# vearch/gamma

Hardware: AMD Instinct MI355X
Metric: queries/sec @ recall@10>=0.95, IVFPQ nlist=4096 nprobe=32 (higher is better)
Workload: dtype f32

## Files before the change

gamma_amd/_lib.py:

```python
import ctypes as C
import os

HERE = os.path.dirname(os.path.abspath(__file__))
LIB_PATH = os.path.join(HERE, "libgamma_hip.so")

f32p = C.POINTER(C.c_float)
i64p = C.POINTER(C.c_int64)
i32p = C.POINTER(C.c_int32)
u8p = C.POINTER(C.c_uint8)

NUM_STAGES = 6
STAGE_NAMES = ["coarse", "tables", "scan", "select", "rerank", "flat"]


class RangeFilter(C.Structure):
    _fields_ = [("bitmap", u8p), ("bitmap_bytes", C.c_int64), ("min_doc", C.c_int32),
                ("max_doc", C.c_int32), ("min_aligned", C.c_int32), ("b_not_in", C.c_int32)]


class FieldFilter(C.Structure):
    _fields_ = [("field_id", C.c_int32), ("include_lower", C.c_int32), ("include_upper", C.c_int32),
                ("reserved", C.c_int32), ("lower_i", C.c_int64), ("upper_i", C.c_int64),
                ("lower_f", C.c_double), ("upper_f", C.c_double)]

# ... 36 lines not shown
    "gamma_hip_raw_i8_check": (C.c_int, [f32p, C.c_int64, C.c_int, i64p]),
    "gamma_hip_raw_init_sq8": (C.c_int, [C.c_void_p, C.c_int]),
    "gamma_hip_raw_sq8_set_ranges": (C.c_int, [C.c_void_p, f32p, f32p]),
    "gamma_hip_raw_sq8_get_ranges": (C.c_int, [C.c_void_p, f32p, f32p]),
    "gamma_hip_raw_sq8_train": (C.c_int, [C.c_void_p, C.c_int64, f32p]),
    "gamma_hip_raw_sq8_check": (C.c_int, [f32p, C.c_int64, i64p]),
    "gamma_hip_raw_sq8_params": (C.c_int, [C.c_int, f32p, f32p, f32p, f32p]),
    "gamma_hip_raw_append": (C.c_int, [C.c_void_p, C.c_int64, f32p]),
    "gamma_hip_raw_update": (C.c_int, [C.c_void_p, C.c_int64, f32p]),
    "gamma_hip_ivfpq_arena_stats": (C.c_int, [C.c_void_p, i64p]),
    "gamma_hip_ivfpq_arena_growth": (C.c_int, [C.c_void_p, i64p]),
    "gamma_hip_ivfpq_set_repack_threshold": (C.c_int, [C.c_void_p, C.c_int64]),
    "gamma_hip_set_small_path": (C.c_int, [C.c_void_p, C.c_int]),
    "gamma_hip_set_flat_narrow_rows": (C.c_int, [C.c_void_p, C.c_int]),
    "gamma_hip_set_ivfflat_narrow_rows": (C.c_int, [C.c_void_p, C.c_int]),
    "gamma_hip_ivfflat_lm_shape": (C.c_int, [C.c_int, C.POINTER(C.c_int), C.POINTER(C.c_int), C.POINTER(C.c_int)]),
    "gamma_hip_ivfflat_scan_stats": (C.c_int, [C.c_void_p, i64p, C.c_int]),
    "gamma_hip_set_flat_sq8_rows": (C.c_int, [C.c_void_p, C.c_int]),
    "gamma_hip_set_ivfflat_sq8_rows": (C.c_int, [C.c_void_p, C.c_int]),
    "gamma_hip_set_coarse_fused": (C.c_int, [C.c_void_p, C.c_int, C.c_int]),
    "gamma_hip_coarse_filter_stats": (C.c_int, [C.c_void_p, i64p]),
    "gamma_hip_set_rerank_filter": (C.c_int, [C.c_void_p, C.c_int]),
    "gamma_hip_rerank_filter_stats": (C.c_int, [C.c_void_p, i64p]),
    "gamma_hip_flat_filter_shape": (C.c_int, [C.c_int, C.POINTER(C.c_int), C.POINTER(C.c_float)]),
    "gamma_hip_flat_filter_stats": (C.c_int, [C.c_void_p, i64p, C.c_int]),
    "gamma_hip_tie_stats": (C.c_int, [C.c_void_p, i64p, C.c_int]),
    "gamma_hip_ties_not_honoured": (C.c_int, [C.c_void_p, i64p, C.c_int]),
    "gamma_hip_blas_form_not_restated": (C.c_int, [C.c_void_p, i64p, C.c_int]),
    "gamma_hip_raw_write": (C.c_int, [C.c_void_p, C.c_int64, C.c_int64, f32p]),
    "gamma_hip_raw_gets": (C.c_int, [C.c_void_p, C.c_int64, i64p, f32p]),
    "gamma_hip_ivfpq_repack_verify_stats": (C.c_int, [C.c_void_p, i64p]),
    "gamma_hip_raw_count": (C.c_int64, [C.c_void_p]),
    "gamma_hip_raw_stats": (C.c_int, [C.c_void_p, i64p]),
    "gamma_hip_bitmap_upload": (C.c_int, [C.c_void_p, u8p, C.c_int64]),
    "gamma_hip_bitmap_set": (C.c_int, [C.c_void_p, i64p, C.c_int64, C.c_int]),
    "gamma_hip_ivfpq_init": (C.c_int, [C.c_void_p] + [C.c_int] * 7),
    "gamma_hip_ivfpq4_init": (C.c_int, [C.c_void_p] + [C.c_int] * 6),
    "gamma_hip_opq_set": (C.c_int, [C.c_void_p, f32p]),
    "gamma_hip_opq_get": (C.c_int, [C.c_void_p, f32p]),
    "gamma_hip_opq_apply": (C.c_int, [C.c_void_p, C.c_int64, f32p, f32p]),
    "gamma_hip_opq_apply_device": (C.c_int, [C.c_void_p, C.c_int64, C.c_void_p, C.c_void_p]),
    "gamma_hip_opq_train": (C.c_int, [C.c_void_p, C.c_int, C.c_int64, f32p, C.c_int, C.c_int, f32p, C.POINTER(C.c_float)]),
    "gamma_hip_ivfpq_set_trained": (C.c_int, [C.c_void_p, f32p, f32p, f32p]),
    "gamma_hip_ivfpq_get_precomputed_table": (C.c_int, [C.c_void_p, f32p]),
    "gamma_hip_set_precomputed_table_max_bytes": (C.c_int, [C.c_int64]),
    "gamma_hip_get_precomputed_table_max_bytes": (C.c_int64, []),
# ... 185 lines not shown
```

gamma_amd/api.py:

```python
import ctypes as C

import numpy as np

from . import _lib
from ._lib import GammaHipError, RangeFilter, SearchParams

METRIC_IP = 0
METRIC_L2 = 1

FLT_TINY = float(np.finfo(np.float32).tiny)
FLT_MAX = float(np.finfo(np.float32).max)


def _f32(a):
    return np.ascontiguousarray(a, dtype=np.float32)


def _p(a, t):
    return a.ctypes.data_as(t) if a is not None else None


def make_range_filter(docids, b_not_in=False):
    docids = np.asarray(sorted(set(int(x) for x in docids)), dtype=np.int64)
    mn, mx = (int(docids[0]), int(docids[-1])) if len(docids) else (0, 0)
# ... 641 lines not shown
        out = np.zeros(4, np.int64)
        self._ck(self.L.gamma_hip_scan_bound_stats(self.h, _p(out, _lib.i64p)), "scan_bound_stats")
        return dict(zip(["fell_through", "queries", "backoffs", "gave_up_waiting"], [int(v) for v in out]))

    def set_dist_budget(self, nbytes):
        self._ck(self.L.gamma_hip_set_workspace_budget(self.h, int(nbytes)), "set_workspace_budget")

    def set_coarse_fused(self, on=True, list_cap=128):
        self._ck(self.L.gamma_hip_set_coarse_fused(self.h, int(on), list_cap), "set_coarse_fused")

    def coarse_filter_stats(self):
        out = np.zeros(4, np.int64)
        self._ck(self.L.gamma_hip_coarse_filter_stats(self.h, _p(out, _lib.i64p)), "coarse_filter_stats")
        return dict(zip(["given_up", "queries", "backoffs", "fp32_calls_left"], [int(v) for v in out]))

    def set_rerank_filter(self, mode=1):
        self._ck(self.L.gamma_hip_set_rerank_filter(self.h, int(mode)), "set_rerank_filter")

    def rerank_filter_stats(self):
        out = np.zeros(5, np.int64)
        self._ck(self.L.gamma_hip_rerank_filter_stats(self.h, _p(out, _lib.i64p)), "rerank_filter_stats")
        return dict(zip(["candidates", "survivors", "calls", "backoffs", "image_rows"], [int(v) for v in out]))

    def flat_filter_stats(self, reset=False):
        out = np.zeros(3, np.int64)
        self._ck(self.L.gamma_hip_flat_filter_stats(self.h, _p(out, _lib.i64p), 1 if reset else 0), "flat_filter_stats")
        return tuple(int(v) for v in out)

    def set_small_path(self, on=True):
        self._ck(self.L.gamma_hip_set_small_path(self.h, int(on)), "set_small_path")

    def set_flat_narrow_rows(self, on=True):
        self._ck(self.L.gamma_hip_set_flat_narrow_rows(self.h, 1 if on else 0), "set_flat_narrow_rows")

    def set_ivfflat_narrow_rows(self, on=True):
        self._ck(self.L.gamma_hip_set_ivfflat_narrow_rows(self.h, 1 if on else 0), "set_ivfflat_narrow_rows")

    def ivfflat_scan_stats(self, reset=False):
        out = np.zeros(4, np.int64)
        self._ck(self.L.gamma_hip_ivfflat_scan_stats(self.h, _p(out, _lib.i64p), 1 if reset else 0), "ivfflat_scan_stats")
        return tuple(int(v) for v in out)

    def set_flat_sq8_rows(self, on=True):
        self._ck(self.L.gamma_hip_set_flat_sq8_rows(self.h, 1 if on else 0), "set_flat_sq8_rows")

    def set_ivfflat_sq8_rows(self, on=True):
# ... 256 lines not shown
```

gamma_amd/csrc/gamma_hip.cpp:

```cpp
#include "gamma_hip_internal.h"

using namespace ghi;

extern "C" {

const char* gamma_hip_strerror(int code) {
    switch (code) {
        case GAMMA_HIP_OK: return "ok";
        case GAMMA_HIP_EINVAL: return "invalid argument";
        case GAMMA_HIP_ENOTTRAINED: return "index not trained";
        case GAMMA_HIP_EDEVICE: return "HIP runtime error";
        case GAMMA_HIP_ENOMEM: return "out of memory";
        case GAMMA_HIP_EFULL: return "inverted list full";
        case GAMMA_HIP_EUNSUPPORTED: return "exact ties requested beyond the replay's range";
        default: return "unknown error";
    }
}

int gamma_hip_create(int device, gamma_hip_index** out) {
    if (!out) return GAMMA_HIP_EINVAL;
    *out = nullptr;
    int ndev = 0;
    if (hipGetDeviceCount(&ndev) != hipSuccess || ndev <= 0) return GAMMA_HIP_EDEVICE;
    if (device < 0 || device >= ndev) return GAMMA_HIP_EINVAL;
// ... 177 lines not shown
    h->rf.mode = mode;
    h->rf.off_calls = 0;
    return GAMMA_HIP_OK;
}

int gamma_hip_rerank_filter_stats(gamma_hip_index* h, int64_t* out5) {
    if (!h || !out5) return GAMMA_HIP_EINVAL;
    SearchLock lk(h);
    std::vector<unsigned long long> v(gh::kRerankFilterStatLines * 16, 0);
    if (h->rf.d_stat) {
        GH_CHECK(h, hipSetDevice(h->device));
        GH_CHECK(h, hipStreamSynchronize(h->stream));
        GH_CHECK(h, hipMemcpy(v.data(), h->rf.d_stat, gh::rerank_filter_stat_bytes(), hipMemcpyDeviceToHost));
    }
    out5[0] = (int64_t)h->rf.cand;
    out5[1] = 0;
    for (int i = 0; i < gh::kRerankFilterStatLines; i++) out5[1] += (int64_t)v[16 * i];
    out5[2] = h->rf.calls;
    out5[3] = h->rf.backoffs;
    out5[4] = h->rf.on ? h->nraw : 0;
    return GAMMA_HIP_OK;
}

int gamma_hip_flat_filter_shape(int d, int* d_pad, float* margin) { return gh::flat_filter_shape(d, d_pad, margin); }

int gamma_hip_flat_filter_stats(gamma_hip_index* h, int64_t* out3, int reset) {
    if (!h || !out3) return GAMMA_HIP_EINVAL;
    out3[0] = reset ? h->ff_passes.exchange(0) : h->ff_passes.load();
    out3[1] = reset ? h->ff_pairs.exchange(0) : h->ff_pairs.load();
    out3[2] = reset ? h->ff_redone.exchange(0) : h->ff_redone.load();
    return GAMMA_HIP_OK;
}

int gamma_hip_ivfflat_lm_shape(int d, int* kind, int* slab, int* qtile) {
    if (!kind || !slab || !qtile) return GAMMA_HIP_EINVAL;
    gh::ivfflat_lm_shape(d, kind, slab, qtile);
    return GAMMA_HIP_OK;
}

int gamma_hip_ivfflat_scan_stats(gamma_hip_index* h, int64_t* out4, int reset) {
    if (!h || !out4) return GAMMA_HIP_EINVAL;
    out4[0] = reset ? h->fl_small.exchange(0) : h->fl_small.load();
    out4[1] = reset ? h->fl_pair.exchange(0) : h->fl_pair.load();
    out4[2] = reset ? h->fl_lm.exchange(0) : h->fl_lm.load();
    out4[3] = reset ? h->fl_lms.exchange(0) : h->fl_lms.load();
    return GAMMA_HIP_OK;
// ... 161 lines not shown
```

gamma_amd/csrc/gamma_hip_internal.h:

```cpp
#pragma once
#include "../../include/gamma_hip.h"

#include <hip/hip_runtime.h>
#include <math.h>
#include <stdlib.h>
#include <string.h>

#include <algorithm>
#include <atomic>
#include <map>
#include <chrono>
#include <condition_variable>
#include <cstring>
#include <deque>
#include <functional>
#include <mutex>
#include <string>
#include <thread>
#include <unordered_map>
#include <vector>

#include "call_slots.h"
#include "dev_mem.h"
#include "kernels.h"
// ... 121 lines not shown
    int64_t raw_cap() const { return raw_d > 0 ? (int64_t)(raw.cap / ((size_t)raw_d * raw_esz())) : 0; }
    std::vector<float> sq8_vmin, sq8_vmax, sq8_step;
    float* d_sq8_tab = nullptr;
    size_t raw_esz() const { return gh::row_elem_bytes(raw_et); }
    bool has_raw_rows() const { return raw.p != nullptr; }
    int raw_elem_type() const { return raw_et; }
    bool raw_narrow() const { return raw_et != gh::ROW_F32; }
    const float* raw_f32() const { return raw_et == gh::ROW_F32 ? static_cast<const float*>(raw.p) : nullptr; }
    float* raw_f32() { return raw_et == gh::ROW_F32 ? static_cast<float*>(raw.p) : nullptr; }
    bool raw_sparse = false;
    std::vector<int32_t> h_raw_slot;
    ghi::DevArrayOf<int32_t> d_raw_slot;
    int64_t raw_slot_cap() const { return (int64_t)(d_raw_slot.cap / sizeof(int32_t)); }
    int64_t raw_live = 0;
    std::vector<int32_t> raw_free;

    struct RerankImage {
        ghi::DevArray rows, aux;
        float* par = nullptr;
        bool on = false;
        hipEvent_t built = nullptr;
        int mode = 1;
        static constexpr int kAutoMinNq = 1024;
        unsigned long long* d_stat = nullptr;
        unsigned long long* pin_stat = nullptr;
        unsigned long long seen[2] = {0, 0};
        unsigned long long cand = 0, cand_at_copy = 0;
        hipEvent_t copy_ev = nullptr;
        bool copy_pending = false;
        uint64_t sig = 0;
        int off_calls = 0;
        int64_t backoffs = 0, calls = 0;
        int64_t cap_rows(int d) const { return d > 0 ? (int64_t)std::min(rows.cap / (size_t)d, aux.cap / (2 * sizeof(float))) : 0; }
    } rf;

    struct Column {
        int dtype = 0;
        ghi::DevArrayOf<uint8_t> d;
        int64_t n = 0;
    };
    std::map<int, Column> fields;
    struct TermColumn {
        ghi::DevArrayOf<int64_t> d_off;
        ghi::DevArrayOf<int32_t> d_tok;
        int64_t ndocs = 0, ntok = 0;
        std::vector<int64_t> h_rows;
// ... 316 lines not shown
```

gamma_amd/csrc/gamma_hip_search.cpp:

```cpp
#include "gamma_hip_internal.h"
#include "gamma_hip_search.h"
#include "opq.h"

namespace ghi {


int build_filter(H* h, const gamma_hip_search_params* p, gh::FilterDesc* f, size_t* off_io, int64_t est_codes) {
    memset(f, 0, sizeof(*f));
    f->del_bitmap = h->d_bitmap;
    f->del_bits = h->d_bitmap ? h->bitmap_bits : 0;
    f->vid2doc = h->h_v2d.empty() ? nullptr : h->d_v2d;
    f->n_vid2doc = (int64_t)h->h_v2d.size();
    f->has_range = p->has_range ? 1 : 0;
    f->n_range = p->has_range ? p->n_range : 0;
    if (f->n_range > gh::kMaxRange) return fail(h, GAMMA_HIP_EINVAL, "too many range filters");
    if (f->n_range > 0) {
        size_t tot = 0;
        for (int i = 0; i < f->n_range; i++) tot += ((size_t)p->range[i].bitmap_bytes + 15) & ~(size_t)15;
        if (!off_io) GH_CHECK(h, h->w_filter.ensure(tot));
        size_t off = off_io ? *off_io : 0;
        for (int i = 0; i < f->n_range; i++) {
            const gamma_hip_range_filter& r = p->range[i];
            uint8_t* dst = h->w_filter.as<uint8_t>() + off;
            GH_CHECK(h, hipMemcpyAsync(dst, r.bitmap, (size_t)r.bitmap_bytes, hipMemcpyHostToDevice,
// ... 725 lines not shown
        a.cand_dis = const_cast<float*>(cand_dis);
        a.cand_ids = const_cast<int64_t*>(cand_ids);
        a.distances = d_distances;
        a.labels = d_labels;
        static const bool no_side = getenv("GAMMA_HIP_NO_SIDE_STREAM") != nullptr;
        if (h->defer_now && h->side2 && !no_side) {
            (void)hipEventRecord(h->ev_rfork, s);
            (void)hipStreamWaitEvent(h->side2, h->ev_rfork, 0);
            gh::launch_tie_replay(h->side2, l2, a);
            (void)hipEventRecord(h->ev_rdone, h->side2);
            h->replay_pending = true;
            h->replay_is_flat = false;
        } else {
            gh::launch_tie_replay(s, l2, a);
        }
    };
    if (p->has_rank) {
        if (!h->has_raw_rows() || h->raw_d != h->d) return fail(h, GAMMA_HIP_EINVAL, "has_rank needs the raw store");
        if (h->raw_sparse) return fail(h, GAMMA_HIP_EUNSUPPORTED, "has_rank on a handle that holds its shard's raw rows only: the exact distances travel with the candidates (gamma_hip_ivfpq_shard_exact / _merge_rerank_exact)");
        if (R <= 1024 && (nq >= 256 || ties)) {
            bool filt = false;
            GH_TRY(rerank_filter_begin(h, l2, nq, R, k, &filt));
            if (filt) {
                gh::launch_rerank_topk_filtered(s, l2, d_x, nq, h->d, h->raw_f32(), h->nraw, h->rf.rows.as<uint8_t>(),
                                                h->rf.aux.as<float>(), h->rf.par, cand_ids, R, k, p->min_score, p->max_score, neutral,
                                                d_distances, d_labels, qperm, ties ? &tf : nullptr, h->rf.d_stat);
                GH_TRY(rerank_filter_end(h, (int64_t)nq * R));
            } else {
                gh::launch_rerank_topk(s, l2, d_x, nq, h->d, raw_rows_ref(h), h->nraw, cand_ids, R, k, p->min_score,
                                       p->max_score, neutral, d_distances, d_labels, qperm, ties ? &tf : nullptr);
            }
            if (ties && tie_mode == 1) replay();
            GH_CHECK(h, hipGetLastError());
            return GAMMA_HIP_OK;
        }
        GH_CHECK(h, h->w_exact.ensure((size_t)nq * R * sizeof(float)));
        GH_CHECK(h, h->w_selv.ensure((size_t)nq * k * sizeof(float)));
        GH_CHECK(h, h->w_selp.ensure((size_t)nq * k * sizeof(int)));
        gh::launch_rerank_dist(s, l2, d_x, nq, h->d, raw_rows_ref(h), h->nraw, cand_ids, R, p->min_score,
                               p->max_score, h->w_exact.as<float>());
        gh::launch_select_topk(s, l2, h->w_exact.as<float>(), R, nullptr, R, R, nq, k,
                               h->w_selv.as<float>(), h->w_selp.as<int>());
        gh::launch_finalize_topk(s, h->w_selv.as<float>(), h->w_selp.as<int>(), nq, k, cand_ids, R, 0,
                                 neutral, d_distances, d_labels);
        if (ties) {
            GH_CHECK(h, h->w_textra.ensure((size_t)nq));
            GH_CHECK(h, hipMemsetAsync(h->w_textra.p, 0, (size_t)nq, s));
            gh::launch_flag_cut_ties(s, h->w_exact.as<float>(), R, nullptr, nq, k, h->w_selv.as<float>(), h->w_selp.as<int>(),
                                     h->w_textra.as<uint8_t>(), R, 1);
// ... 527 lines not shown
```

gamma_amd/csrc/kernels.h:

```cpp
#pragma once
#include <atomic>
#include <hip/hip_runtime.h>
#include <stdint.h>

#include "scan_plan.h"

namespace gh {

void launch_refused(const char* what);
const char* launch_refused_take();


inline bool first_call_on_device(std::atomic<uint64_t>& done) {
    int dev = 0;
    (void)hipGetDevice(&dev);
    const uint64_t bit = 1ull << (dev & 63);
    return (done.fetch_or(bit) & bit) == 0;
}

constexpr int kMaxRange = 8;

struct RangeDesc {
    const uint8_t* bitmap;
    int32_t min_doc, max_doc, min_aligned, b_not_in;
// ... 327 lines not shown
                         const float* vals, const int64_t* ids, int64_t stride, const int32_t* off, int P, const float* bound, float* ex);
void launch_lookup_exact(hipStream_t s, bool l2, const float* all_dis, const int64_t* all_ids, const float* all_exact, int W, int nq, int R,
                         int q0, int nql, const float* cand_dis, const int64_t* cand_ids, float* cand_exact);
struct TieFlags {
    const uint8_t* cut = nullptr;
    int* list = nullptr;
    int* count = nullptr;
    unsigned long long* stats = nullptr;
};
void launch_rerank_topk(hipStream_t s, bool l2, const float* x, int nq, int d, const RowsRef& raw,
                        int64_t nraw, const int64_t* cand_ids, int R, int k, float min_score,
                        float max_score, float neutral, float* distances, int64_t* labels,
                        const int* qperm = nullptr,
                        const TieFlags* ties = nullptr);
constexpr float kRerankFilterMargin = 3.0517578125e-05f;
constexpr int kRerankFilterMaxD = 1536;
constexpr int kRerankFilterStatLines = 64;
inline size_t rerank_filter_stat_bytes() { return (size_t)kRerankFilterStatLines * 16 * sizeof(unsigned long long); }
bool rerank_filter_shape_ok(int d, int R, int k);
inline size_t rerank_image_par_bytes(int d) { return ((size_t)3 * d + 2) * sizeof(float); }
void launch_rerank_image_params(hipStream_t s, const float* rows, int64_t n, int d, float* par);
void launch_rerank_image_rows(hipStream_t s, const float* rows, const int64_t* vids, int64_t first, int64_t n, int d, const float* par,
                              uint8_t* img, float* aux, int64_t nrows);
void launch_rerank_topk_filtered(hipStream_t s, bool l2, const float* x, int nq, int d, const float* raw, int64_t nraw, const uint8_t* img,
                                 const float* aux, const float* par, const int64_t* cand_ids, int R, int k, float min_score,
                                 float max_score, float neutral, float* distances, int64_t* labels, const int* qperm,
                                 const TieFlags* ties, unsigned long long* stat);
struct TieReplayArgs {
    const int* list;
    const int* count;
    int nq;
    const float* slab;
    int64_t q_stride;
    const int* pair_off;
    const int64_t* pair_base;
    const int64_t* ids;
    int P, G;
    const unsigned long long* ready;
    const unsigned long long* surv;
    const int* gcnt;
    int nsl, slice_cap;
    const float* x;
    int d;
    RowsRef rows;
    int64_t nraw;
    const float* ex_slab = nullptr;
    int* ex_missing = nullptr;
    int R, k, has_rank;
    float min_score, max_score, neutral;
    float* cand_dis;
// ... 73 lines not shown
```

gamma_amd/csrc/rerank_filter.hip:

```cpp
#include <hip/hip_runtime.h>
#include <stdint.h>

#include <algorithm>

#include "block_utils.h"
#include "device_math.h"
#include "kernels.h"
#include "rerank_dev.h"
#include "rerank_topk_dev.h"

namespace gh {

namespace {
constexpr float kM = kRerankFilterMargin;

__device__ __forceinline__ float group8_sum(float a) {
    a += __shfl_down(a, 4, 8);
    a += __shfl_down(a, 2, 8);
    return a + __shfl_down(a, 1, 8);
}
__device__ __forceinline__ float byte_f(uint32_t w, int b) { return (float)((w >> (8 * b)) & 0xffu); }

__device__ __forceinline__ float block_sum256(float v, float* red) {
#pragma unroll
    for (int o = 32; o > 0; o >>= 1) v += __shfl_down(v, o, 64);
    __syncthreads();
    if ((threadIdx.x & 63) == 0) red[threadIdx.x >> 6] = v;
    __syncthreads();
    return (red[0] + red[1]) + (red[2] + red[3]);
}
}

__global__ __launch_bounds__(256) void k_img_minmax_init(uint32_t* __restrict__ keys, int d) {
    const int j = blockIdx.x * 256 + threadIdx.x;
    if (j < d) {
        keys[j] = 0xffffffffu;
        keys[d + j] = 0u;
    }
}
__global__ __launch_bounds__(256) void k_img_minmax(const float* __restrict__ rows, int64_t n, int d, uint32_t* __restrict__ keys) {
    __shared__ uint32_t s_lo[4][64], s_hi[4][64];
    const int tx = threadIdx.x & 63, ty = threadIdx.x >> 6;
    const int j = blockIdx.x * 64 + tx;
    uint32_t lo = 0xffffffffu, hi = 0u;
    if (j < d)
        for (int64_t r = (int64_t)blockIdx.y * 4 + ty; r < n; r += (int64_t)gridDim.y * 4) {
            const float v = rows[r * d + j];
            if (fabsf(v) < INFINITY) {
                const uint32_t kk = f2key(v);
                lo = min(lo, kk);
                hi = max(hi, kk);
            }
        }
// ... 100 lines not shown
        launch_refused("launch_rerank_image_rows: d is not a multiple of 16");
        return;
    }
    hipLaunchKernelGGL(k_img_quantise, dim3((unsigned)((n + 31) / 32)), dim3(256), 0, s, rows, vids, first, n, d, par, img,
                       reinterpret_cast<float2*>(aux), nrows);
}

template <bool L2, bool D128>
__global__ __launch_bounds__(256) void k_rerank_topk_filt(const float* __restrict__ x, int d, const float* __restrict__ raw, int64_t nraw,
                                                          const uint8_t* __restrict__ img, const float2* __restrict__ aux,
                                                          const float* __restrict__ par, const int64_t* __restrict__ cand_ids, int R,
                                                          int k, float min_score, float max_score, float neutral,
                                                          float* __restrict__ distances, int64_t* __restrict__ labels, int nq,
                                                          const int* __restrict__ qperm, TieFlags tf,
                                                          unsigned long long* __restrict__ stat) {
    __shared__ unsigned long long s_it[1024];
    __shared__ int64_t s_id[1024];
    __shared__ float s_bd[1024];
    __shared__ unsigned short s_sv[1024];
    __shared__ __attribute__((aligned(16))) float s_x[D128 ? 128 : kRerankFilterMaxD];
    __shared__ float s_red[4];
    __shared__ float s_tau;
    __shared__ int s_tie, s_nsv;
    int q = blockIdx.x;
    if (qperm) {
        const int qi = (blockIdx.x & 7) * ((nq + 7) >> 3) + (blockIdx.x >> 3);
        if (qi >= nq) return;
        q = qperm[qi];
    } else if (q >= nq) {
        return;
    }
    const int l = threadIdx.x & 7, g = threadIdx.x >> 3;
    const float* xq = x + (int64_t)q * d;
    const float sentinel = L2 ? INFINITY : -INFINITY;
    const float delta = par[d], lon = par[d + 1];
    for (int r = threadIdx.x; r < R; r += 256) s_id[r] = cand_ids[(int64_t)q * R + r];
    if (threadIdx.x == 0) s_nsv = 0;
    float sq = 0.f, sc = 0.f;
    for (int j = threadIdx.x; j < d; j += 256) {
        const float xv = xq[j];
        const float v = L2 ? __fsub_rn(xv, par[j]) : xv;
        s_x[j] = v;
        sq = __builtin_fmaf(v, v, sq);
        if (!L2) sc = __builtin_fmaf(xv, par[j], sc);
    }
    const float xn = sqrtf(block_sum256(sq, s_red)) * (1.0f + kM);
    float c0 = 0.f;
    if (!L2) c0 = block_sum256(sc, s_red);

    if constexpr (D128) {
        float xx[16];
#pragma unroll
        for (int u = 0; u < 16; u++) xx[u] = s_x[16 * l + u];
        for (int r0 = 0; r0 < R; r0 += 128) {
            uint4 w[4];
#pragma unroll
            for (int f = 0; f < 4; f++) {
                const int r = r0 + 32 * f + g;
                const int64_t id = r < R ? s_id[r] : -1;
                w[f] = make_uint4(0, 0, 0, 0);
#if GH_RERANK_TIMING == 5
                w[f] = make_uint4((uint32_t)id, l, f, 7);
#else
                if (id >= 0 && id < nraw) w[f] = *reinterpret_cast<const uint4*>(img + id * 128 + 16 * l);
#endif
            }
#pragma unroll
            for (int f = 0; f < 4; f++) {
                const uint32_t ww[4] = {w[f].x, w[f].y, w[f].z, w[f].w};
                float a = 0.f;
#pragma unroll
// ... 24 lines not shown
                    const uint32_t ww[4] = {w.x, w.y, w.z, w.w};
#pragma unroll
                    for (int v = 0; v < 4; v++) {
                        const float4 xv = *reinterpret_cast<const float4*>(s_x + 16 * c + 4 * v);
                        const float xs[4] = {xv.x, xv.y, xv.z, xv.w};
#pragma unroll
                        for (int b = 0; b < 4; b++) {
                            const float uf = byte_f(ww[v], b);
                            if (L2) {
                                const float t = __builtin_fmaf(-delta, uf, xs[b]);
                                a = __builtin_fmaf(t, t, a);
                            } else {
                                a = __builtin_fmaf(xs[b], uf, a);
                            }
                        }
                    }
                }
            }
            a = group8_sum(a);
            if (l == 0 && r < R) s_bd[r] = a;
        }
    }
    __syncthreads();
    float bd[4];
    bool alive[4];
#pragma unroll
    for (int u = 0; u < 4; u++) {
        const int r = threadIdx.x + 256 * u;
        bd[u] = 0.f;
        alive[u] = false;
        if (r < R) {
            const int64_t id = s_id[r];
            const bool live = id >= 0 && id < nraw;
            float2 ax = make_float2(0.f, 0.f);
#if GH_RERANK_TIMING == 2
            if (live) ax = make_float2(0.1f, 1000.0f);
#else
            if (live) ax = aux[id];
#endif
            const float a = s_bd[r];
            float lb, ub;
            if (L2) {
                const float rt = sqrtf(a);
                const float slack = __builtin_fmaf(kM, rt + xn, ax.x);
                const float ur = rt + slack, lr = fmaxf(rt - slack, 0.0f);
                ub = ur * ur * (1.0f + kM);
                lb = lr * lr * (1.0f - kM);
            } else {
                const float est = __builtin_fmaf(delta, a, c0);
                const float slack = xn * __builtin_fmaf(kM, ax.y + lon, ax.x);
                ub = est + slack;
                lb = est - slack;
            }
            const bool inside = live && ub <= max_score && lb >= min_score;
            alive[u] = live && !(lb > max_score || ub < min_score);
            const uint32_t key = L2 ? f2key(ub) : ~f2key(lb);
            s_it[r] = inside ? (((unsigned long long)key << 32) | (unsigned)r) : ~0ull;
            bd[u] = L2 ? lb : ub;
        }
    }
    if (threadIdx.x == 0) {
        if (tf.list) s_tie = tf.cut ? tf.cut[q] : 0;
        s_tau = sentinel;
    }
    const int K1 = min(k + 1, R);
    const bool head = K1 <= 16 && R > 64;
    if (head) {
        __syncthreads();
        if (threadIdx.x < 64) {
            const unsigned long long it = wave_sort64(s_it[threadIdx.x]);
            const uint32_t key = (uint32_t)(it >> 32);
            if ((int)threadIdx.x == K1 - 1 && key != 0xffffffffu) s_tau = key2f(L2 ? key : ~key);
        }
    } else {
        rerank_first_k(s_it, R, K1);
        if (threadIdx.x == 0) {
            const uint32_t key = (uint32_t)(s_it[K1 - 1] >> 32);
            if (key != 0xffffffffu) s_tau = key2f(L2 ? key : ~key);
        }
    }
    __syncthreads();
    const float tau = s_tau;
    const uint32_t skey = L2 ? f2key(sentinel) : ~f2key(sentinel);
    bool sv[4];
#pragma unroll
    for (int u = 0; u < 4; u++) sv[u] = alive[u] && !(L2 ? bd[u] > tau : bd[u] < tau);
#pragma unroll
    for (int u = 0; u < 4; u++) {
        const int r = threadIdx.x + 256 * u;
        if (256 * u < R) {
            const unsigned long long bal = __ballot(sv[u]);
            const int lane = threadIdx.x & 63;
            int base = 0;
            if (lane == 0 && bal) base = atomicAdd(&s_nsv, __popcll(bal));
            base = __shfl(base, 0, 64);
            if (sv[u]) s_sv[base + __popcll(bal & ((1ull << lane) - 1ull))] = (unsigned short)r;
            else if (r < R) s_it[r] = ((unsigned long long)skey << 32) | (unsigned)r;
        }
    }
    __syncthreads();
#if GH_RERANK_TIMING == 3
    const int m = 0;
#else
    const int m = s_nsv;
#endif
#if GH_RERANK_TIMING != 4
    if (threadIdx.x == 0 && stat) atomicAdd(stat + 16 * (blockIdx.x & (kRerankFilterStatLines - 1)), (unsigned long long)m);
#endif

    auto put = [&](int r, float dis) {
        if (l == 0) {
            if (!(dis <= max_score && dis >= min_score)) dis = sentinel;
            const uint32_t key = L2 ? f2key(dis) : ~f2key(dis);
            s_it[r] = ((unsigned long long)key << 32) | (unsigned)r;
        }
    };
    if constexpr (D128) {
        float xx[16];
#pragma unroll
        for (int u = 0; u < 16; u++) xx[u] = xq[l + 8 * u];
        for (int c0_ = 0; c0_ < m; c0_ += 32) {
            if (c0_ + (g & ~7) >= m) continue;
            const int c = c0_ + g;
// ... 8 lines not shown
            for (int u = 0; u < 16; u++) {
                if (L2) {
                    const float t = xx[u] - fa[u];
                    a = __builtin_fmaf(t, t, a);
                } else {
                    a = __builtin_fmaf(xx[u], fa[u], a);
                }
            }
            const float sa = __shfl_down(a, 4, 8) + a;
            const float ta = sa + __shfl_down(sa, 1, 8);
            const float da = ta + __shfl_down(ta, 2, 8);
            if (live) put(r, da);
        }
    } else {
        for (int c0_ = 0; c0_ < m; c0_ += 32) {
            if (c0_ + (g & ~7) >= m) continue;
            const int c = c0_ + g;
            const bool live = c < m;
            const int r = live ? s_sv[c] : 0;
            const float dis = rerank_dist8<L2>(xq, raw + (live ? s_id[r] : 0) * d, d, l, live);
            if (live) put(r, dis);
        }
    }
    if (m <= 64) {
        __syncthreads();
        if (threadIdx.x < 64) {
            const unsigned long long it = wave_sort64((int)threadIdx.x < m ? s_it[s_sv[threadIdx.x]] : ~0ull);
            if ((int)threadIdx.x < K1) s_it[threadIdx.x] = it != ~0ull ? it : ((unsigned long long)skey << 32);
        }
        __syncthreads();
    } else {
        rerank_first_k(s_it, R, K1);
    }
    rerank_topk_out<L2>(s_it, s_id, &s_tie, q, R, k, neutral, distances, labels, tf);
}

bool rerank_filter_shape_ok(int d, int R, int k) { return d > 0 && d % 16 == 0 && d <= kRerankFilterMaxD && R >= 1 && R <= 1024 && std::min(k + 1, R) <= 64; }

void launch_rerank_topk_filtered(hipStream_t s, bool l2, const float* x, int nq, int d, const float* raw, int64_t nraw, const uint8_t* img,
                                 const float* aux, const float* par, const int64_t* cand_ids, int R, int k, float min_score,
                                 float max_score, float neutral, float* distances, int64_t* labels, const int* qperm,
                                 const TieFlags* ties, unsigned long long* stat) {
    if (nq <= 0) return;
    if (!rerank_filter_shape_ok(d, R, k) || nraw <= 0) {
        launch_refused("launch_rerank_topk_filtered: a shape its caller rules out");
        return;
    }
    const TieFlags tf = ties ? *ties : TieFlags{};
    const dim3 grid((unsigned)(8 * ((nq + 7) / 8)));
    const float2* ax = reinterpret_cast<const float2*>(aux);
#define GH_FILT(L2_, D128_)                                                                                                          \
    hipLaunchKernelGGL((k_rerank_topk_filt<L2_, D128_>), grid, dim3(256), 0, s, x, d, raw, nraw, img, ax, par, cand_ids, R, k,      \
                       min_score, max_score, neutral, distances, labels, nq, qperm, tf, stat)
    if (d == 128) {
        if (l2) GH_FILT(true, true);
        else GH_FILT(false, true);
    } else {
        if (l2) GH_FILT(true, false);
        else GH_FILT(false, false);
    }
#undef GH_FILT
}

}
```

gamma_amd/csrc/rerank_topk_dev.h:

```cpp
#pragma once
#include <hip/hip_runtime.h>
#include <stdint.h>

#include "block_utils.h"
#include "device_math.h"
#include "kernels.h"

namespace gh {

__device__ __forceinline__ void rerank_first_k(unsigned long long* s_it, int R, int K1) {
    if (K1 <= 64) {
        const int w = threadIdx.x >> 6, lane = threadIdx.x & 63;
        const int nruns = (R + 63) >> 6;
        __syncthreads();
        for (int run = w; run < nruns; run += 4) {
            const int idx = run * 64 + lane;
            s_it[idx] = wave_sort64(idx < R ? s_it[idx] : ~0ull);
        }
        __syncthreads();
        unsigned long long xr[4];
        int rkk[4];
#pragma unroll
        for (int u = 0; u < 4; u++) {
            const int run = w + 4 * u;
// ... 50 lines not shown
        __syncthreads();
        if (threadIdx.x == 0 && *s_tie) {
            tf.list[atomicAdd(tf.count, 1)] = q;
            if (tf.stats) atomicAdd(tf.stats + 2, 1ull);
        }
    }
    for (int i = threadIdx.x; i < k; i += 256) {
        float val = neutral;
        int64_t id = -1;
        if (i < R) {
            const unsigned long long it = s_it[i];
            const uint32_t key = (uint32_t)(it >> 32);
            const float dv = key2f(L2 ? key : ~key);
            if (dv != sentinel) {
                val = dv;
                id = s_id[(uint32_t)it];
            }
        }
        distances[(int64_t)q * k + i] = val;
        labels[(int64_t)q * k + i] = id;
    }
}

}
```

include/gamma_hip.h:

```cpp
#ifndef GAMMA_HIP_H_
#define GAMMA_HIP_H_

#include <stddef.h>
#include <stdint.h>

#ifdef __cplusplus
extern "C" {
#endif

#define GAMMA_HIP_METRIC_IP 0
#define GAMMA_HIP_METRIC_L2 1

#define GAMMA_HIP_OK 0
#define GAMMA_HIP_EINVAL (-1)
#define GAMMA_HIP_ENOTTRAINED (-2)
#define GAMMA_HIP_EDEVICE (-3)
#define GAMMA_HIP_ENOMEM (-4)
#define GAMMA_HIP_EFULL (-5)
#define GAMMA_HIP_EUNSUPPORTED (-6)

typedef struct gamma_hip_index gamma_hip_index;

typedef struct {
    const uint8_t* bitmap;
// ... 40 lines not shown
    const gamma_hip_range_filter* range;
    int32_t n_field;
    int32_t n_term;
    const gamma_hip_field_filter* field;
    const gamma_hip_term_filter* term;
    int32_t exact_ties;
} gamma_hip_search_params;

int gamma_hip_create(int device, gamma_hip_index** out);
int gamma_hip_destroy(gamma_hip_index* h);
const char* gamma_hip_strerror(int code);
const char* gamma_hip_last_error(gamma_hip_index* h);
void* gamma_hip_stream(gamma_hip_index* h);
int gamma_hip_synchronize(gamma_hip_index* h);

int gamma_hip_set_scan_bound_feedback(gamma_hip_index* h, int on);
int gamma_hip_scan_bound_stats(gamma_hip_index* h, int64_t* out4);
int gamma_hip_set_workspace_budget(gamma_hip_index* h, int64_t bytes);
int gamma_hip_set_exact_ties(gamma_hip_index* h, int on);
int gamma_hip_set_coarse_fused(gamma_hip_index* h, int on, int list_cap);
int gamma_hip_coarse_filter_stats(gamma_hip_index* h, int64_t* out4);
int gamma_hip_set_rerank_filter(gamma_hip_index* h, int mode);
int gamma_hip_rerank_filter_stats(gamma_hip_index* h, int64_t* out5);
int gamma_hip_flat_filter_shape(int d, int* d_pad, float* margin);
int gamma_hip_flat_filter_stats(gamma_hip_index* h, int64_t* out3, int reset);
int gamma_hip_set_small_path(gamma_hip_index* h, int on);
int gamma_hip_set_flat_narrow_rows(gamma_hip_index* h, int on);
int gamma_hip_set_ivfflat_narrow_rows(gamma_hip_index* h, int on);
int gamma_hip_ivfflat_lm_shape(int d, int* kind, int* slab, int* qtile);
int gamma_hip_ivfflat_scan_stats(gamma_hip_index* h, int64_t* out4, int reset);
int gamma_hip_set_flat_sq8_rows(gamma_hip_index* h, int on);
int gamma_hip_set_ivfflat_sq8_rows(gamma_hip_index* h, int on);
int gamma_hip_tie_stats(gamma_hip_index* h, int64_t* out3, int reset);
int gamma_hip_ties_not_honoured(gamma_hip_index* h, int64_t* out_calls, int reset);
int gamma_hip_blas_form_not_restated(gamma_hip_index* h, int64_t* out_calls, int reset);

int gamma_hip_field_append(gamma_hip_index* h, int field_id, int dtype, int64_t n, const void* values);
int gamma_hip_field_update(gamma_hip_index* h, int field_id, int64_t docid, const void* value);
int64_t gamma_hip_field_count(gamma_hip_index* h, int field_id);
int gamma_hip_term_append(gamma_hip_index* h, int field_id, int64_t n_docs, const int32_t* counts,
                          const int32_t* items);
int64_t gamma_hip_term_count(gamma_hip_index* h, int field_id);
int gamma_hip_term_update(gamma_hip_index* h, int field_id, int64_t docid, int32_t count, const int32_t* items);

int gamma_hip_raw_init(gamma_hip_index* h, int d);
int gamma_hip_raw_append(gamma_hip_index* h, int64_t n, const float* vecs);
// ... 250 lines not shown
```

Measured before the change: 12.13 million.

## Add single-wavefront filtered rerank kernel for d=128 with auto selection at large nq

Adds a 64-thread, one-wavefront-per-query variant of the filtered rerank top-k kernel for d=128 and R<=256. It uses wave shuffles, ballots and wave-level sorts instead of 256-thread block reductions and __syncthreads. The launcher picks it automatically when nq>=4096, or when the new form knob forces it. The aim is to cut block-level sync overhead and raise occupancy. The cost is less parallelism per query and more registers per lane. Also adds optional per-phase clock instrumentation compiled only under a timing macro.

```diff
diff --git a/gamma_amd/_lib.py b/gamma_amd/_lib.py
--- a/gamma_amd/_lib.py
+++ b/gamma_amd/_lib.py
@@ -82,6 +82,8 @@
     "gamma_hip_coarse_filter_stats": (C.c_int, [C.c_void_p, i64p]),
     "gamma_hip_set_rerank_filter": (C.c_int, [C.c_void_p, C.c_int]),
     "gamma_hip_rerank_filter_stats": (C.c_int, [C.c_void_p, i64p]),
+    "gamma_hip_set_rerank_filter_form": (C.c_int, [C.c_void_p, C.c_int]),
+    "gamma_hip_rerank_filter_form": (C.c_int, [C.c_void_p, i64p]),
     "gamma_hip_flat_filter_shape": (C.c_int, [C.c_int, C.POINTER(C.c_int), C.POINTER(C.c_float)]),
     "gamma_hip_flat_filter_stats": (C.c_int, [C.c_void_p, i64p, C.c_int]),
     "gamma_hip_tie_stats": (C.c_int, [C.c_void_p, i64p, C.c_int]),
diff --git a/gamma_amd/api.py b/gamma_amd/api.py
--- a/gamma_amd/api.py
+++ b/gamma_amd/api.py
@@ -687,6 +687,14 @@
         self._ck(self.L.gamma_hip_rerank_filter_stats(self.h, _p(out, _lib.i64p)), "rerank_filter_stats")
         return dict(zip(["candidates", "survivors", "calls", "backoffs", "image_rows"], [int(v) for v in out]))
 
+    def set_rerank_filter_form(self, form=0):
+        self._ck(self.L.gamma_hip_set_rerank_filter_form(self.h, int(form)), "set_rerank_filter_form")
+
+    def rerank_filter_form(self):
+        out = np.zeros(4, np.int64)
+        self._ck(self.L.gamma_hip_rerank_filter_form(self.h, _p(out, _lib.i64p)), "rerank_filter_form")
+        return dict(zip(["form", "last", "wave_calls", "auto_min_nq"], [int(v) for v in out]))
+
     def flat_filter_stats(self, reset=False):
         out = np.zeros(3, np.int64)
         self._ck(self.L.gamma_hip_flat_filter_stats(self.h, _p(out, _lib.i64p), 1 if reset else 0), "flat_filter_stats")
diff --git a/gamma_amd/csrc/gamma_hip.cpp b/gamma_amd/csrc/gamma_hip.cpp
--- a/gamma_amd/csrc/gamma_hip.cpp
+++ b/gamma_amd/csrc/gamma_hip.cpp
@@ -223,6 +223,23 @@
     return GAMMA_HIP_OK;
 }
 
+int gamma_hip_set_rerank_filter_form(gamma_hip_index* h, int form) {
+    if (!h || form < 0 || form > 2) return GAMMA_HIP_EINVAL;
+    SearchLock lk(h);
+    h->rf.form = form;
+    return GAMMA_HIP_OK;
+}
+
+int gamma_hip_rerank_filter_form(gamma_hip_index* h, int64_t* out4) {
+    if (!h || !out4) return GAMMA_HIP_EINVAL;
+    SearchLock lk(h);
+    out4[0] = h->rf.form;
+    out4[1] = h->rf.last_form;
+    out4[2] = h->rf.wave_calls;
+    out4[3] = gh::kRerankWaveAutoMinNq;
+    return GAMMA_HIP_OK;
+}
+
 int gamma_hip_flat_filter_shape(int d, int* d_pad, float* margin) { return gh::flat_filter_shape(d, d_pad, margin); }
 
 int gamma_hip_flat_filter_stats(gamma_hip_index* h, int64_t* out3, int reset) {
diff --git a/gamma_amd/csrc/gamma_hip_internal.h b/gamma_amd/csrc/gamma_hip_internal.h
--- a/gamma_amd/csrc/gamma_hip_internal.h
+++ b/gamma_amd/csrc/gamma_hip_internal.h
@@ -167,6 +167,9 @@
         hipEvent_t built = nullptr;
         int mode = 1;
         static constexpr int kAutoMinNq = 1024;
+        int form = 0;
+        int last_form = 0;
+        int64_t wave_calls = 0;
         unsigned long long* d_stat = nullptr;
         unsigned long long* pin_stat = nullptr;
         unsigned long long seen[2] = {0, 0};
diff --git a/gamma_amd/csrc/gamma_hip_search.cpp b/gamma_amd/csrc/gamma_hip_search.cpp
--- a/gamma_amd/csrc/gamma_hip_search.cpp
+++ b/gamma_amd/csrc/gamma_hip_search.cpp
@@ -771,9 +771,12 @@
             bool filt = false;
             GH_TRY(rerank_filter_begin(h, l2, nq, R, k, &filt));
             if (filt) {
-                gh::launch_rerank_topk_filtered(s, l2, d_x, nq, h->d, h->raw_f32(), h->nraw, h->rf.rows.as<uint8_t>(),
-                                                h->rf.aux.as<float>(), h->rf.par, cand_ids, R, k, p->min_score, p->max_score, neutral,
-                                                d_distances, d_labels, qperm, ties ? &tf : nullptr, h->rf.d_stat);
+                const int ran = gh::launch_rerank_topk_filtered(s, l2, d_x, nq, h->d, h->raw_f32(), h->nraw, h->rf.rows.as<uint8_t>(),
+                                                                h->rf.aux.as<float>(), h->rf.par, cand_ids, R, k, p->min_score,
+                                                                p->max_score, neutral, d_distances, d_labels, qperm,
+                                                                ties ? &tf : nullptr, h->rf.d_stat, h->rf.form);
+                if (ran) h->rf.last_form = ran;
+                if (ran == 2) h->rf.wave_calls++;
                 GH_TRY(rerank_filter_end(h, (int64_t)nq * R));
             } else {
                 gh::launch_rerank_topk(s, l2, d_x, nq, h->d, raw_rows_ref(h), h->nraw, cand_ids, R, k, p->min_score,
diff --git a/gamma_amd/csrc/kernels.h b/gamma_amd/csrc/kernels.h
--- a/gamma_amd/csrc/kernels.h
+++ b/gamma_amd/csrc/kernels.h
@@ -373,10 +373,12 @@
 void launch_rerank_image_params(hipStream_t s, const float* rows, int64_t n, int d, float* par);
 void launch_rerank_image_rows(hipStream_t s, const float* rows, const int64_t* vids, int64_t first, int64_t n, int d, const float* par,
                               uint8_t* img, float* aux, int64_t nrows);
-void launch_rerank_topk_filtered(hipStream_t s, bool l2, const float* x, int nq, int d, const float* raw, int64_t nraw, const uint8_t* img,
+bool rerank_filter_wave_ok(int d, int R, int k);
+constexpr int kRerankWaveAutoMinNq = 4096;
+int launch_rerank_topk_filtered(hipStream_t s, bool l2, const float* x, int nq, int d, const float* raw, int64_t nraw, const uint8_t* img,
                                  const float* aux, const float* par, const int64_t* cand_ids, int R, int k, float min_score,
                                  float max_score, float neutral, float* distances, int64_t* labels, const int* qperm,
-                                 const TieFlags* ties, unsigned long long* stat);
+                                 const TieFlags* ties, unsigned long long* stat, int form = 0);
 struct TieReplayArgs {
     const int* list;
     const int* count;
diff --git a/gamma_amd/csrc/rerank_filter.hip b/gamma_amd/csrc/rerank_filter.hip
--- a/gamma_amd/csrc/rerank_filter.hip
+++ b/gamma_amd/csrc/rerank_filter.hip
@@ -1,5 +1,8 @@
 #include <hip/hip_runtime.h>
 #include <stdint.h>
+#if GH_RERANK_TIMING == 6
+#include <stdio.h>
+#endif
 
 #include <algorithm>
 
@@ -29,6 +32,17 @@
     __syncthreads();
     return (red[0] + red[1]) + (red[2] + red[3]);
 }
+
+#if GH_RERANK_TIMING == 6
+__device__ unsigned long long g_phase_clk[16];
+#define GH_CLK_DECL unsigned long long clk[9]; const bool clk_on = threadIdx.x == 0 && (blockIdx.x & 15) == 0
+#define GH_CLK(i) do { if (clk_on) clk[i] = wall_clock64(); } while (0)
+#define GH_CLK_END do { if (clk_on) { for (int i_ = 0; i_ < 8; i_++) atomicAdd(g_phase_clk + i_, clk[i_ + 1] - clk[i_]); atomicAdd(g_phase_clk + 15, 1ull); } } while (0)
+#else
+#define GH_CLK_DECL
+#define GH_CLK(i)
+#define GH_CLK_END
+#endif
 }
 
 __global__ __launch_bounds__(256) void k_img_minmax_init(uint32_t* __restrict__ keys, int d) {
@@ -175,6 +189,8 @@
     __shared__ float s_red[4];
     __shared__ float s_tau;
     __shared__ int s_tie, s_nsv;
+    GH_CLK_DECL;
+    GH_CLK(0);
     int q = blockIdx.x;
     if (qperm) {
         const int qi = (blockIdx.x & 7) * ((nq + 7) >> 3) + (blockIdx.x >> 3);
@@ -200,6 +216,7 @@
     const float xn = sqrtf(block_sum256(sq, s_red)) * (1.0f + kM);
     float c0 = 0.f;
     if (!L2) c0 = block_sum256(sc, s_red);
+    GH_CLK(1);
 
     if constexpr (D128) {
         float xx[16];
@@ -270,6 +287,7 @@
         }
     }
     __syncthreads();
+    GH_CLK(2);
     float bd[4];
     bool alive[4];
 #pragma unroll
@@ -307,6 +325,7 @@
             bd[u] = L2 ? lb : ub;
         }
     }
+    GH_CLK(3);
     if (threadIdx.x == 0) {
         if (tf.list) s_tie = tf.cut ? tf.cut[q] : 0;
         s_tau = sentinel;
@@ -329,6 +348,7 @@
     }
     __syncthreads();
     const float tau = s_tau;
+    GH_CLK(4);
     const uint32_t skey = L2 ? f2key(sentinel) : ~f2key(sentinel);
     bool sv[4];
 #pragma unroll
@@ -347,6 +367,7 @@
         }
     }
     __syncthreads();
+    GH_CLK(5);
 #if GH_RERANK_TIMING == 3
     const int m = 0;
 #else
@@ -401,6 +422,7 @@
             if (live) put(r, dis);
         }
     }
+    GH_CLK(6);
     if (m <= 64) {
         __syncthreads();
         if (threadIdx.x < 64) {
@@ -411,23 +433,275 @@
     } else {
         rerank_first_k(s_it, R, K1);
     }
+    GH_CLK(7);
     rerank_topk_out<L2>(s_it, s_id, &s_tie, q, R, k, neutral, distances, labels, tf);
-}
+    GH_CLK(8);
+    GH_CLK_END;
+}
+
+constexpr int kRerankWaveMaxR = 256;
+
+__device__ __forceinline__ float wave_sum_first(float v) {
+#pragma unroll
+    for (int o = 32; o > 0; o >>= 1) v += __shfl_down(v, o, 64);
+    return __uint_as_float(__builtin_amdgcn_readfirstlane(__float_as_uint(v)));
+}
+
+template <bool L2>
+__global__ __launch_bounds__(64) void k_rerank_topk_filt_wave(const float* __restrict__ x, const float* __restrict__ raw, int64_t nraw,
+                                                                   const uint8_t* __restrict__ img, const float2* __restrict__ aux,
+                                                                   const float* __restrict__ par, const int64_t* __restrict__ cand_ids,
+                                                                   int R, int k, float min_score, float max_score, float neutral,
+                                                                   float* __restrict__ distances, int64_t* __restrict__ labels, int nq,
+                                                                   const int* __restrict__ qperm, TieFlags tf,
+                                                                   unsigned long long* __restrict__ stat) {
+    __shared__ int64_t s_id[kRerankWaveMaxR];
+    __shared__ uint32_t s_bd[kRerankWaveMaxR];
+    __shared__ unsigned short s_sv[kRerankWaveMaxR];
+    GH_CLK_DECL;
+    GH_CLK(0);
+    const int lane = threadIdx.x;
+    int q = blockIdx.x;
+    if (qperm) {
+        const int qi = (blockIdx.x & 7) * ((nq + 7) >> 3) + (blockIdx.x >> 3);
+        if (qi >= nq) return;
+        q = qperm[qi];
+    } else if (q >= nq) {
+        return;
+    }
+    const int l = lane & 7, g = lane >> 3;
+    const float* xq = x + (int64_t)q * 128;
+    const float sentinel = L2 ? INFINITY : -INFINITY;
+    const uint32_t skey = L2 ? f2key(sentinel) : ~f2key(sentinel);
+    const int K1 = min(k + 1, R);
+    float4 xv4[4], lo4[4];
+    float xh[2], loh[2];
+#pragma unroll
+    for (int v = 0; v < 4; v++) {
+        xv4[v] = *reinterpret_cast<const float4*>(xq + 16 * l + 4 * v);
+        lo4[v] = L2 ? *reinterpret_cast<const float4*>(par + 16 * l + 4 * v) : make_float4(0.f, 0.f, 0.f, 0.f);
+    }
+#pragma unroll
+    for (int h = 0; h < 2; h++) xh[h] = xq[lane + 64 * h], loh[h] = par[lane + 64 * h];
+    const float delta = par[128], lon = par[129];
+    bool live[4];
+    float2 ax[4];
+#pragma unroll
+    for (int u = 0; u < 4; u++) {
+        const int r = lane + 64 * u;
+        const int64_t id = r < R ? cand_ids[(int64_t)q * R + r] : -1;
+        if (64 * u < R) s_id[r] = id;
+        live[u] = id >= 0 && id < nraw;
+        ax[u] = make_float2(0.f, 0.f);
+        if (live[u]) ax[u] = aux[id];
+    }
+    int tie = 0;
+    if (tf.list && tf.cut) tie = tf.cut[q];
+    float xx[16];
+#pragma unroll
+    for (int v = 0; v < 4; v++) {
+        xx[4 * v] = xv4[v].x, xx[4 * v + 1] = xv4[v].y, xx[4 * v + 2] = xv4[v].z, xx[4 * v + 3] = xv4[v].w;
+        if (L2) {
+            xx[4 * v] = __fsub_rn(xv4[v].x, lo4[v].x), xx[4 * v + 1] = __fsub_rn(xv4[v].y, lo4[v].y);
+            xx[4 * v + 2] = __fsub_rn(xv4[v].z, lo4[v].z), xx[4 * v + 3] = __fsub_rn(xv4[v].w, lo4[v].w);
+        }
+    }
+    float sq[2], sc[2];
+#pragma unroll
+    for (int h = 0; h < 2; h++) {
+        const float v = L2 ? __fsub_rn(xh[h], loh[h]) : xh[h];
+        sq[h] = wave_sum_first(__builtin_fmaf(v, v, 0.f));
+        sc[h] = L2 ? 0.f : wave_sum_first(__builtin_fmaf(xh[h], loh[h], 0.f));
+    }
+    const float xn = sqrtf((sq[0] + sq[1]) + 0.f) * (1.0f + kM);
+    const float c0 = L2 ? 0.f : (sc[0] + sc[1]) + 0.f;
+    wave_lds_sync();
+    GH_CLK(1);
+
+    for (int r0 = 0; r0 < R; r0 += 32) {
+        uint4 w[4];
+#pragma unroll
+        for (int f = 0; f < 4; f++) {
+            const int r = r0 + 8 * f + g;
+            const int64_t id = r < R ? s_id[r] : -1;
+            w[f] = make_uint4(0, 0, 0, 0);
+            if (id >= 0 && id < nraw) w[f] = *reinterpret_cast<const uint4*>(img + id * 128 + 16 * l);
+        }
+#pragma unroll
+        for (int f = 0; f < 4; f++) {
+            const uint32_t ww[4] = {w[f].x, w[f].y, w[f].z, w[f].w};
+            float a = 0.f;
+#pragma unroll
+            for (int u = 0; u < 16; u++) {
+                const float uf = byte_f(ww[u >> 2], u & 3);
+                if (L2) {
+                    const float t = __builtin_fmaf(-delta, uf, xx[u]);
+                    a = __builtin_fmaf(t, t, a);
+                } else {
+                    a = __builtin_fmaf(xx[u], uf, a);
+                }
+            }
+            a = group8_sum(a);
+            if (l == 0 && r0 + 8 * f + g < R) s_bd[r0 + 8 * f + g] = __float_as_uint(a);
+        }
+    }
+    wave_lds_sync();
+    GH_CLK(2);
+    unsigned long long it[4];
+    float bd[4];
+    bool alive[4];
+#pragma unroll
+    for (int u = 0; u < 4; u++) {
+        const int r = lane + 64 * u;
+        it[u] = ~0ull;
+        bd[u] = 0.f;
+        alive[u] = false;
+        if (r < R) {
+            const float a = __uint_as_float(s_bd[r]);
+            float lb, ub;
+            if (L2) {
+                const float rt = sqrtf(a);
+                const float slack = __builtin_fmaf(kM, rt + xn, ax[u].x);
+                const float ur = rt + slack, lr = fmaxf(rt - slack, 0.0f);
+                ub = ur * ur * (1.0f + kM);
+                lb = lr * lr * (1.0f - kM);
+            } else {
+                const float est = __builtin_fmaf(delta, a, c0);
+                const float slack = xn * __builtin_fmaf(kM, ax[u].y + lon, ax[u].x);
+                ub = est + slack;
+                lb = est - slack;
+            }
+            const bool inside = live[u] && ub <= max_score && lb >= min_score;
+            alive[u] = live[u] && !(lb > max_score || ub < min_score);
+            const uint32_t key = L2 ? f2key(ub) : ~f2key(lb);
+            if (inside) it[u] = ((unsigned long long)key << 32) | (unsigned)r;
+            bd[u] = L2 ? lb : ub;
+        }
+    }
+    GH_CLK(3);
+    uint32_t tkey;
+    if ((K1 <= 16 && R > 64) || R <= 64) {
+        tkey = (uint32_t)(wave_sort64(it[0]) >> 32);
+    } else {
+        unsigned long long t4[4] = {it[0], it[1], it[2], it[3]};
+        wave_sort_net<4>(t4);
+        tkey = (uint32_t)(t4[0] >> 32);
+    }
+    tkey = (uint32_t)__shfl((int)tkey, K1 - 1, 64);
+    const float tau = tkey != 0xffffffffu ? key2f(L2 ? tkey : ~tkey) : sentinel;
+    GH_CLK(4);
+    bool sv[4];
+    int m = 0;
+#pragma unroll
+    for (int u = 0; u < 4; u++) {
+        const int r = lane + 64 * u;
+        sv[u] = alive[u] && !(L2 ? bd[u] > tau : bd[u] < tau);
+        it[u] = r < R ? (((unsigned long long)skey << 32) | (unsigned)r) : ~0ull;
+        if (64 * u < R) {
+            const unsigned long long bal = __ballot(sv[u]);
+            if (sv[u]) s_sv[m + __popcll(bal & ((1ull << lane) - 1ull))] = (unsigned short)r;
+            m += __popcll(bal);
+        }
+    }
+    if (lane == 0 && stat) atomicAdd(stat + 16 * (blockIdx.x & (kRerankFilterStatLines - 1)), (unsigned long long)m);
+    wave_lds_sync();
+    GH_CLK(5);
+
+    {
+        float x2[16];
+#pragma unroll
+        for (int u = 0; u < 16; u++) x2[u] = xq[l + 8 * u];
+        for (int c0_ = 0; c0_ < m; c0_ += 8) {
+            const int c = c0_ + g;
+            const bool on = c < m;
+            const int r = on ? s_sv[c] : 0;
+            const float* v = raw + (on ? s_id[r] : 0) * 128 + l;
+            float fa[16];
+#pragma unroll
+            for (int u = 0; u < 16; u++) fa[u] = v[8 * u];
+            float a = 0.f;
+#pragma unroll
+            for (int u = 0; u < 16; u++) {
+                if (L2) {
+                    const float t = x2[u] - fa[u];
+                    a = __builtin_fmaf(t, t, a);
+                } else {
+                    a = __builtin_fmaf(x2[u], fa[u], a);
+                }
+            }
+            const float sa = __shfl_down(a, 4, 8) + a;
+            const float ta = sa + __shfl_down(sa, 1, 8);
+            float dis = ta + __shfl_down(ta, 2, 8);
+            if (on && l == 0) {
+                if (!(dis <= max_score && dis >= min_score)) dis = sentinel;
+                s_bd[r] = L2 ? f2key(dis) : ~f2key(dis);
+            }
+        }
+    }
+    wave_lds_sync();
+    GH_CLK(6);
+    unsigned long long first;
+    if (m <= 64) {
+        unsigned long long mine = ~0ull;
+        if (lane < m) {
+            const unsigned r = s_sv[lane];
+            mine = ((unsigned long long)s_bd[r] << 32) | r;
+        }
+        mine = wave_sort64(mine);
+        first = mine != ~0ull ? mine : ((unsigned long long)skey << 32);
+    } else {
+#pragma unroll
+        for (int u = 0; u < 4; u++)
+            if (sv[u]) it[u] = ((unsigned long long)s_bd[lane + 64 * u] << 32) | (unsigned)(lane + 64 * u);
+        wave_sort_net<4>(it);
+        first = it[0];
+    }
+    GH_CLK(7);
+    rerank_topk_out_wave<L2>(first, s_id, tie, q, R, k, neutral, distances, labels, tf);
+    GH_CLK(8);
+    GH_CLK_END;
+}
+
+bool rerank_filter_wave_ok(int d, int R, int k) { return d == 128 && R >= 1 && R <= kRerankWaveMaxR && std::min(k + 1, R) <= 64; }
 
 bool rerank_filter_shape_ok(int d, int R, int k) { return d > 0 && d % 16 == 0 && d <= kRerankFilterMaxD && R >= 1 && R <= 1024 && std::min(k + 1, R) <= 64; }
 
-void launch_rerank_topk_filtered(hipStream_t s, bool l2, const float* x, int nq, int d, const float* raw, int64_t nraw, const uint8_t* img,
-                                 const float* aux, const float* par, const int64_t* cand_ids, int R, int k, float min_score,
-                                 float max_score, float neutral, float* distances, int64_t* labels, const int* qperm,
-                                 const TieFlags* ties, unsigned long long* stat) {
-    if (nq <= 0) return;
-    if (!rerank_filter_shape_ok(d, R, k) || nraw <= 0) {
+int launch_rerank_topk_filtered(hipStream_t s, bool l2, const float* x, int nq, int d, const float* raw, int64_t nraw, const uint8_t* img,
+                                const float* aux, const float* par, const int64_t* cand_ids, int R, int k, float min_score,
+                                float max_score, float neutral, float* distances, int64_t* labels, const int* qperm,
+                                const TieFlags* ties, unsigned long long* stat, int form) {
+    if (nq <= 0) return 0;
+    if (!rerank_filter_shape_ok(d, R, k) || nraw <= 0 || form < 0 || form > 2) {
         launch_refused("launch_rerank_topk_filtered: a shape its caller rules out");
-        return;
+        return 0;
     }
     const TieFlags tf = ties ? *ties : TieFlags{};
+    const float2* ax = reinterpret_cast<const float2*>(aux);
+#if GH_RERANK_TIMING == 6
+#ifdef GH_RERANK_TIMING_FORM
+    form = GH_RERANK_TIMING_FORM;
+#endif
+    static int timed_launches = 0;
+    if (++timed_launches % 20 == 0) {
+        unsigned long long v[16];
+        if (hipStreamSynchronize(s) == hipSuccess && hipMemcpyFromSymbol(v, HIP_SYMBOL(g_phase_clk), sizeof(v)) == hipSuccess && v[15]) {
+            fprintf(stderr, "rerank phase clocks, form %d, %llu workgroups, mean ticks of 10 ns:", form, v[15]);
+            for (int i = 0; i < 8; i++) fprintf(stderr, " %.1f", (double)v[i] / (double)v[15]);
+            fprintf(stderr, "\n");
+        }
+    }
+#endif
+    if (rerank_filter_wave_ok(d, R, k) && (form == 2 || (form == 0 && nq >= kRerankWaveAutoMinNq))) {
+        const dim3 grid((unsigned)(8 * ((nq + 7) / 8)));
+#define GH_FILT_WAVE(L2_)                                                                                                            \
+    hipLaunchKernelGGL((k_rerank_topk_filt_wave<L2_>), grid, dim3(64), 0, s, x, raw, nraw, img, ax, par, cand_ids, R, k, min_score,  \
+                       max_score, neutral, distances, labels, nq, qperm, tf, stat)
+        if (l2) GH_FILT_WAVE(true);
+        else GH_FILT_WAVE(false);
+#undef GH_FILT_WAVE
+        return 2;
+    }
     const dim3 grid((unsigned)(8 * ((nq + 7) / 8)));
-    const float2* ax = reinterpret_cast<const float2*>(aux);
 #define GH_FILT(L2_, D128_)                                                                                                          \
     hipLaunchKernelGGL((k_rerank_topk_filt<L2_, D128_>), grid, dim3(256), 0, s, x, d, raw, nraw, img, ax, par, cand_ids, R, k,      \
                        min_score, max_score, neutral, distances, labels, nq, qperm, tf, stat)
@@ -439,6 +713,7 @@
         else GH_FILT(false, false);
     }
 #undef GH_FILT
-}
-
-}
+    return 1;
+}
+
+}
diff --git a/gamma_amd/csrc/rerank_topk_dev.h b/gamma_amd/csrc/rerank_topk_dev.h
--- a/gamma_amd/csrc/rerank_topk_dev.h
+++ b/gamma_amd/csrc/rerank_topk_dev.h
@@ -96,4 +96,41 @@
     }
 }
 
+__device__ __forceinline__ void wave_lds_sync() {
+    __builtin_amdgcn_fence(__ATOMIC_RELEASE, "wavefront");
+    __builtin_amdgcn_wave_barrier();
+    __builtin_amdgcn_fence(__ATOMIC_ACQUIRE, "wavefront");
 }
+template <bool L2>
+__device__ __forceinline__ void rerank_topk_out_wave(unsigned long long item, const int64_t* s_id, int tie, int q, int R, int k,
+                                                     float neutral, float* __restrict__ distances, int64_t* __restrict__ labels,
+                                                     const TieFlags& tf) {
+    const float sentinel = L2 ? INFINITY : -INFINITY;
+    const int lane = threadIdx.x & 63;
+    if (tf.list) {
+        const unsigned long long next = __shfl_down(item, 1, 64);
+        const uint32_t ka = (uint32_t)(item >> 32), kb = (uint32_t)(next >> 32);
+        const bool eq = lane < k && lane + 1 < R && ka == kb && ka != (L2 ? f2key(sentinel) : ~f2key(sentinel));
+        if (__ballot(eq)) tie = 1;
+        if (lane == 0 && tie) {
+            tf.list[atomicAdd(tf.count, 1)] = q;
+            if (tf.stats) atomicAdd(tf.stats + 2, 1ull);
+        }
+    }
+    for (int i = lane; i < k; i += 64) {
+        float val = neutral;
+        int64_t id = -1;
+        if (i < R) {
+            const uint32_t key = (uint32_t)(item >> 32);
+            const float dv = key2f(L2 ? key : ~key);
+            if (dv != sentinel) {
+                val = dv;
+                id = s_id[(uint32_t)item];
+            }
+        }
+        distances[(int64_t)q * k + i] = val;
+        labels[(int64_t)q * k + i] = id;
+    }
+}
+
+}
diff --git a/include/gamma_hip.h b/include/gamma_hip.h
--- a/include/gamma_hip.h
+++ b/include/gamma_hip.h
@@ -86,6 +86,8 @@
 int gamma_hip_coarse_filter_stats(gamma_hip_index* h, int64_t* out4);
 int gamma_hip_set_rerank_filter(gamma_hip_index* h, int mode);
 int gamma_hip_rerank_filter_stats(gamma_hip_index* h, int64_t* out5);
+int gamma_hip_set_rerank_filter_form(gamma_hip_index* h, int form);
+int gamma_hip_rerank_filter_form(gamma_hip_index* h, int64_t* out4);
 int gamma_hip_flat_filter_shape(int d, int* d_pad, float* margin);
 int gamma_hip_flat_filter_stats(gamma_hip_index* h, int64_t* out3, int reset);
 int gamma_hip_set_small_path(gamma_hip_index* h, int on);
```

Result: faster. 12.41 million (median of 6 runs) (+2.3%).
